# OpenGene/gencore

Hardware: AMD Instinct MI355X
Metric: consensus read-pairs/sec (whole node) + clustering HBM GB/s vs roofline (higher is better)
Workload: dtype u8

## Files before the change

### gencore_amd/csrc/engine.hip

```cpp
#include <hip/hip_runtime.h>
#include <hip/hip_ext.h>
#include <cstdio>
#include <cstdlib>
#include <algorithm>
#include <cstring>
#include <ctime>
#include <string>
#include <vector>

#include "gce_kernels.hpp"
#include "gce_pair2.hpp"
#include "gce_vote.hpp"
#include "gce_deep.hpp"
#include "gce_output.hpp"
#include "gce_depth.hpp"
#include "gce_inflate.hpp"
#include "gce_deflate.hpp"

namespace {

static thread_local double t_alloc_s = 0.0; static thread_local long t_alloc_n = 0; static thread_local size_t t_alloc_bytes = 0;
static inline double mono_s() { struct timespec ts; clock_gettime(CLOCK_MONOTONIC, &ts); return (double)ts.tv_sec + 1e-9 * (double)ts.tv_nsec; }
long long g_dev_live = 0, g_dev_peak = 0;
static int64_t g_pass_idx_ctr[4] = {0, 0, 0, 0};
// ... 466 lines not shown
    return GCE_OK;
}

__global__ __launch_bounds__(256) void k_publish_si(const StreamInfo *si, StreamInfo *host, unsigned long long *flag, unsigned long long seq) {
    const uint32_t *src = reinterpret_cast<const uint32_t *>(si);
    uint32_t *dst = reinterpret_cast<uint32_t *>(host);
    for (unsigned i = threadIdx.x; i < sizeof(StreamInfo) / 4; i += 256) dst[i] = src[i];
    __threadfence_system();
    __syncthreads();
    if (threadIdx.x == 0) __hip_atomic_store(flag, seq, __ATOMIC_RELEASE, __HIP_MEMORY_SCOPE_SYSTEM);
}
static_assert(sizeof(StreamInfo) % 4 == 0, "k_publish_si copies words");
static int read_si_begin(gce_engine *e, unsigned long long *seq_out) {
    *seq_out = 0;
    static const bool sync_copy = getenv("GCE_SYNC_COPY") != nullptr;
    if (!sync_copy && !e->si_pin) {
        void *hp = nullptr;
        if (hipHostMalloc(&hp, sizeof(StreamInfo) + 64, hipHostMallocMapped | hipHostMallocCoherent | hipHostMallocPortable) == hipSuccess) {
            void *dp = nullptr;
            if (hipHostGetDevicePointer(&dp, hp, 0) == hipSuccess) { memset(hp, 0, sizeof(StreamInfo) + 64); e->si_pin = hp; e->si_pin_dev = dp; }
            else (void)hipHostFree(hp);
        }
        (void)hipGetLastError();
    }
    if (!sync_copy && e->si_pin) {
        unsigned long long *dflag = reinterpret_cast<unsigned long long *>(reinterpret_cast<char *>(e->si_pin_dev) + ((sizeof(StreamInfo) + 7) & ~size_t(7)));
        const unsigned long long seq = ++e->si_seq;
        hipLaunchKernelGGL(k_publish_si, dim3(1), dim3(256), 0, e->stream, (const StreamInfo *)e->si.p, reinterpret_cast<StreamInfo *>(e->si_pin_dev), dflag, seq);
        HIPCHK(hipGetLastError());
        *seq_out = seq;
    }
    return GCE_OK;
}
static int read_si_end(gce_engine *e, unsigned long long seq) {
    bool published = false;
    if (seq) {
        StreamInfo *hs = reinterpret_cast<StreamInfo *>(e->si_pin);
        unsigned long long *hflag = reinterpret_cast<unsigned long long *>(reinterpret_cast<char *>(e->si_pin) + ((sizeof(StreamInfo) + 7) & ~size_t(7)));
        for (unsigned spins = 1;; spins++) {
            if (__atomic_load_n(hflag, __ATOMIC_ACQUIRE) == seq) { published = true; break; }
            if ((spins & 0x3FFF) == 0) {
                const hipError_t q = hipStreamQuery(e->stream);
                if (q == hipSuccess) { published = __atomic_load_n(hflag, __ATOMIC_ACQUIRE) == seq; break; }
                if (q != hipErrorNotReady) HIPCHK(q);
            }
            __builtin_ia32_pause();
        }
        if (published) memcpy(&e->h_si, hs, sizeof(StreamInfo));
    }
    if (!published) {
        HIPCHK(hipMemcpyAsync(&e->h_si, e->si.p, sizeof(StreamInfo), hipMemcpyDeviceToHost, e->stream));
        HIPCHK(hipStreamSynchronize(e->stream));
    }
    for (int k = 0; k < 6; k++) for (int q = 0; q < GCE_PRE_SLOTS; q++) { e->h_si.pre[k] += e->h_si.pre_slot[q][k]; e->h_si.post[k] += e->h_si.post_slot[q][k]; }
    if (e->h_si.err_key != ~0ull) { e->dev_error = -(int)(e->h_si.err_key & 0xFF); e->dev_error_read = (uint32_t)(e->h_si.err_key >> 8); }
    return GCE_OK;
}
static int read_si(gce_engine *e) {
    unsigned long long seq = 0;
    const int rc = read_si_begin(e, &seq);
    return rc != GCE_OK ? rc : read_si_end(e, seq);
}

static inline unsigned cdiv(uint64_t a, uint64_t b) { return (unsigned)((a + b - 1) / b); }
static const bool g_record_events = getenv("GCE_RECORD_EVENTS") != nullptr;
#define LAUNCH_EV(kernel, grid, block, stream, ev, ...) do { \
    if (g_record_events) { hipLaunchKernelGGL(kernel, grid, block, 0, stream, __VA_ARGS__); (void)hipEventRecord(ev, stream); } \
    else hipExtLaunchKernelGGL(kernel, grid, block, 0, stream, nullptr, ev, 0, __VA_ARGS__); } while (0)

struct FillSeg { void *p; uint64_t bytes; uint32_t val; uint32_t pad; };
struct FillArgs { FillSeg s[6]; };
__global__ __launch_bounds__(256) void k_fill_many(FillArgs a) {
    const FillSeg g = a.s[blockIdx.y];
    const uint64_t n16 = g.bytes >> 4;
    const uint32_t v = g.val * 0x01010101u;
    uint4 *q = reinterpret_cast<uint4 *>(g.p);
    for (uint64_t i = (uint64_t)blockIdx.x * 256 + threadIdx.x; i < n16; i += (uint64_t)gridDim.x * 256) q[i] = make_uint4(v, v, v, v);
    if (blockIdx.x == 0 && threadIdx.x < (g.bytes & 15)) reinterpret_cast<uint8_t *>(g.p)[(n16 << 4) + threadIdx.x] = (uint8_t)g.val;
}
static void fill_many(hipStream_t s, std::initializer_list<FillSeg> segs) {
    FillArgs a{}; int n = 0; uint64_t mx = 0;
    for (const FillSeg &g : segs) { a.s[n++] = g; mx = std::max<uint64_t>(mx, g.bytes); }
    const unsigned gx = (unsigned)std::min<uint64_t>(std::max<uint64_t>((mx >> 4) / (256 * 8), 1), 2048);
    hipLaunchKernelGGL(k_fill_many, dim3(gx, (unsigned)n), dim3(256), 0, s, a);
}

static int aux_ready(gce_engine *e) {
    if (e->aux_stream) return GCE_OK;
// ... 139 lines not shown
        int cb = 1; while (cb < 33 && (1ull << cb) <= (uint64_t)N + 1024) cb++;
        int qb = 1; while (qb < 52 && (1ull << qb) <= qmax) qb++;
        p.nw_cb = cb; p.nw_bd = 62 - cb - qb; p.nw_ok = !e->target_len.empty() && p.nw_bd >= 1;
        if (p.nw_bd > 40) p.nw_bd = 40;
    }
    const size_t qual_bytes = hb.qual_bytes ? hb.qual_bytes : 1;
    const size_t nsb1 = (size_t)(n_sblk > 0 ? n_sblk : 1);
#define ENS(buf, bytes) HIPCHK(e->buf.ensure(bytes))
    ENS(uinfo, n1 * 8); ENS(rdesc, n1 * sizeof(ReadDescP)); ENS(spatch, n1 * 4); ENS(slot, n1 * 4 + 16); ENS(score, qual_bytes + 64);
    ENS(out_flag, n1 + 144);        ENS(nmx, n1 * 4); ENS(orec, n1 * sizeof(OutRec)); ENS(out_index, n1 * 4);
    ENS(lrec, nsb1 * SB_READS * sizeof(LeadRec)); ENS(lout, nsb1 * SB_READS * sizeof(LeadOut));
    ENS(bhdr, nsb1 * sizeof(BlkHdr)); ENS(blk_base, nsb1 * 4);
    ENS(ev_tid, (size_t)max_events * 4); ENS(ev_pos, (size_t)max_events * 4); ENS(ev_read, (size_t)max_events * 4);
    ENS(table, T * sizeof(TabEntry)); ENS(toff, T * 4);
    ENS(k64, n1 * 24); ENS(members, n1 * 4); ENS(sorted, n1 * 4); ENS(pl, n1 * 4); ENS(pr, n1 * 4); ENS(pu, n1 * 4); ENS(pg, n1 * 4); ENS(gpl, n1 * 4); ENS(gpr, n1 * 4);
    ENS(grp_begin, n1 * 4); ENS(grp_n, n1 * 4); ENS(slow_list, n1 * 4 + 64);
    w.slow_list = e->slow_list.as<uint32_t>();
    ENS(deep_list, (n1 / 64 + 64) * 16); w.deep_list = e->deep_list.p;
    const unsigned nblk_N = cdiv(n1, SCAN_TILE);
    ENS(scan_part, std::max<size_t>(2 * nsb1, (size_t)2 * nblk_N) * 8 + 16);     ENS(si, sizeof(StreamInfo));
    w.uinfo = e->uinfo.as<uint64_t>(); w.rdesc = e->rdesc.as<ReadDescP>(); w.spatch = e->spatch.as<uint32_t>();
    w.slot = e->slot.as<uint32_t>(); w.score = e->score.as<int8_t>();
    w.out_flag = e->out_flag.as<uint8_t>(); w.nmx = e->nmx.as<uint32_t>(); w.orec = e->orec.as<OutRec>(); w.out_index = e->out_index.as<uint32_t>();
    w.lrec = e->lrec.as<LeadRec>(); w.lout = e->lout.as<LeadOut>(); w.bhdr = e->bhdr.as<BlkHdr>(); w.blk_base = e->blk_base.as<uint32_t>();
    w.ev_tid = e->ev_tid.as<int32_t>(); w.ev_pos = e->ev_pos.as<int32_t>(); w.ev_read = e->ev_read.as<uint32_t>();
    w.tab = e->table.as<TabEntry>(); w.toff = e->toff.as<uint32_t>();
    w.k64 = e->k64.as<uint64_t>(); w.members = e->members.as<uint32_t>(); w.sorted = e->sorted.as<uint32_t>(); w.pl = e->pl.as<uint32_t>(); w.pr = e->pr.as<uint32_t>();
    w.pu = e->pu.as<uint32_t>(); w.pg = e->pg.as<uint32_t>(); w.gpl = e->gpl.as<uint32_t>(); w.gpr = e->gpr.as<uint32_t>();
    w.grp_begin = e->grp_begin.as<uint32_t>(); w.grp_n = e->grp_n.as<uint32_t>();
    w.scan_part = e->scan_part.as<uint64_t>(); w.si = e->si.as<StreamInfo>();
    ENS(cl_ikey, n1 * 4); ENS(cl_start, n1 * 4); ENS(cl_n, n1 * 4);
    w.cl_ikey = e->cl_ikey.as<uint32_t>(); w.cl_start = e->cl_start.as<uint32_t>(); w.cl_n = e->cl_n.as<uint32_t>();

    StreamInfo init{}; init.first_unmapped = NONE32; init.err_key = ~0ull; init.lq_min = 0x7FFFFFFF; init.lq_max = -1;
    if (e->have_tick) { init.n_events = init.n_events_a = (int)e->h_ev_tid.size(); }
    HIPCHK(hipMemcpyAsync(e->si.p, &init, sizeof init, hipMemcpyHostToDevice, e->stream));
    if (e->have_tick && !e->h_ev_tid.empty()) {
        HIPCHK(hipMemcpyAsync(e->ev_tid.p, e->h_ev_tid.data(), e->h_ev_tid.size() * 4, hipMemcpyHostToDevice, e->stream));
        HIPCHK(hipMemcpyAsync(e->ev_pos.p, e->h_ev_pos.data(), e->h_ev_pos.size() * 4, hipMemcpyHostToDevice, e->stream));
    }
    hipStream_t s = e->stream;
    if (!e->tab_clean || e->tab_clean_ptr != e->table.p || e->tab_clean_cap != e->table.cap) {
        HIPCHK(hipMemsetAsync(e->table.p, 0, e->table.cap, s));
        e->tab_clean_ptr = e->table.p; e->tab_clean_cap = e->table.cap;
    }
    e->tab_clean = false;
    HIPCHK(hipEventRecord(e->ev[EV_START], s));
    HIPCHK(hipMemsetAsync(e->out_flag.p, 0, n1, s));
    if (N > 0) LAUNCH_EV(k_cluster, dim3((unsigned)n_sblk), dim3(SB_T), s, e->ev[EV_CLUSTER], b, p, w);
#ifdef CL_PROF
    if (N > 0) {
        StreamInfo hs; (void)hipStreamSynchronize(s); (void)hipMemcpy(&hs, e->si.p, sizeof hs, hipMemcpyDeviceToHost);
        static const char *nm[3] = {"key records + keys", "LDS leaders", "stores"};
        const double blocks = (double)hs.prof[15];
        fprintf(stderr, "k_cluster phases, mean per block (us), %.0f blocks:", blocks);
        for (int k = 0; k < 3; k++) fprintf(stderr, " %s %.2f;", nm[k], blocks ? hs.prof[k] / blocks / 100.0 : 0.0);
        fprintf(stderr, "\n");
    }
#endif
    if (N <= 0) HIPCHK(hipEventRecord(e->ev[EV_CLUSTER], s));
    CANARY("EV_CLUSTER");
    if (N > 0) {
        if (!e->have_tick) {
            hipLaunchKernelGGL(k_blk_scan, dim3(1), dim3(1024), 0, s, w, p);
            hipLaunchKernelGGL(k_events, dim3(cdiv(max_events, EV_T / 64)), dim3(EV_T), 0, s, b, p, w);
        }
        const unsigned nb4 = cdiv(n_sblk, 4);
        hipLaunchKernelGGL(k_leaders, dim3(nb4), dim3(256), 0, s, b, p, w);
        hipLaunchKernelGGL(k_num_reduce, dim3(nb4), dim3(256), 0, s, w, p.nw_cb);
        hipLaunchKernelGGL(k_scan_partials, dim3(1), dim3(1024), 0, s, w.scan_part, (uint64_t)nb4, &w.si->n_clusters, (unsigned long long *)nullptr);
        hipLaunchKernelGGL(k_num_apply, dim3(nb4), dim3(256), 0, s, w);
        LAUNCH_EV(k_scatter, dim3((unsigned)n_sblk), dim3(SB_T), s, e->ev[EV_CSR], N, w);
    } else HIPCHK(hipEventRecord(e->ev[EV_CSR], s));
    CANARY("EV_CSR");
    unsigned long long si_seq1 = 0;
    if ((rc = read_si_begin(e, &si_seq1)) != GCE_OK) return rc;
    if (N > 0) {
#ifndef GCE_DESCRIBE_BLOCKS
#define GCE_DESCRIBE_BLOCKS 32768
#endif
        const int64_t n_tiles = (N + 255) / 256;
        int tpb = (int)((n_tiles + GCE_DESCRIBE_BLOCKS - 1) / GCE_DESCRIBE_BLOCKS); if (tpb < 1) tpb = 1;
        LAUNCH_EV(k_describe, dim3(cdiv(n_tiles, tpb)), dim3(256), s, e->ev[EV_DESCRIBE], b, p, w, tpb);
    } else HIPCHK(hipEventRecord(e->ev[EV_DESCRIBE], s));
    CANARY("EV_DESCRIBE");
    if ((rc = read_si_end(e, si_seq1)) != GCE_OK) return rc;
    HIPCHK(hipGetLastError());
    e->tab_clean = true;
    const uint32_t C = (uint32_t)e->h_si.n_clusters;
    const size_t c1 = C ? C : 1;
    ENS(cl_npairs, c1 * 4); ENS(cl_ngroups, c1 * 4); ENS(cl_gbase, c1 * 4); ENS(cl_nresult, c1 * 4); ENS(cl_hasumi, c1); ENS(cl_tier, c1);
    w.cl_npairs = e->cl_npairs.as<uint32_t>(); w.cl_ngroups = e->cl_ngroups.as<uint32_t>(); w.cl_gbase = e->cl_gbase.as<uint32_t>();
    w.cl_nresult = e->cl_nresult.as<uint32_t>(); w.cl_hasumi = e->cl_hasumi.as<uint8_t>(); w.cl_tier = e->cl_tier.as<uint8_t>();
    uint32_t NG = 0;
    bool si_behind_describe = false;
    if (C > 0 && e->dev_error == 0) {
        ENS(left_list, c1 * 4 + 64); w.left_list = e->left_list.as<uint32_t>();
        ENS(pf_flag, c1 + 64); ENS(pf_list, c1 * 4); ENS(pq_flag, c1 + 64); ENS(pq_list, c1 * 4); ENS(p16_flag, c1 + 64); ENS(p16_list, c1 * 4);
        w.pf_flag = e->pf_flag.as<uint8_t>(); w.pf_list = e->pf_list.as<uint32_t>(); w.pq_flag = e->pq_flag.as<uint8_t>(); w.pq_list = e->pq_list.as<uint32_t>(); w.p16_flag = e->p16_flag.as<uint8_t>(); w.p16_list = e->p16_list.as<uint32_t>();
        const bool pair_classes = (double)N > 10.0 * (double)C;
        if (!pair_classes) fill_many(s, {FillSeg{e->pf_flag.p, c1, 0u, 0u}, FillSeg{e->pq_flag.p, c1, 0u, 0u}});
        const unsigned nbc = cdiv(C, SCAN_TILE);
        auto compact = [&](uint8_t *flag, uint32_t *list, unsigned long long *count) {
            hipLaunchKernelGGL(k_flag_reduce, dim3(nbc), dim3(256), 0, s, (const uint8_t *)flag, (uint64_t)C, w.scan_part);
            hipLaunchKernelGGL(k_scan_partials, dim3(1), dim3(1024), 0, s, w.scan_part, (uint64_t)nbc, count, (unsigned long long *)nullptr);
            hipLaunchKernelGGL(k_flag_apply, dim3(nbc), dim3(256), 0, s, (const uint8_t *)flag, (uint64_t)C, (const uint64_t *)w.scan_part, list);
        };
#ifdef PS_STOP
        {
            hipEvent_t a_, b_, c_; (void)hipEventCreate(&a_); (void)hipEventCreate(&b_); (void)hipEventCreate(&c_);
            (void)hipEventRecord(a_, s);
            hipLaunchKernelGGL(k_pairing_sub<16>, dim3(cdiv(C, 4 * WAVES_PER_BLOCK)), dim3(256), 0, s, b, p, w, C, (const uint32_t *)nullptr, (const unsigned long long *)nullptr, w.pq_flag, 0);
            (void)hipEventRecord(b_, s);
            hipLaunchKernelGGL(k_pairing_sub<32>, dim3(cdiv(C, 2 * WAVES_PER_BLOCK)), dim3(256), 0, s, b, p, w, C, (const uint32_t *)nullptr, (const unsigned long long *)nullptr, w.pf_flag, 0);
            (void)hipEventRecord(c_, s); (void)hipEventSynchronize(c_);
            float m1 = 0, m2 = 0; (void)hipEventElapsedTime(&m1, a_, b_); (void)hipEventElapsedTime(&m2, b_, c_);
            fprintf(stderr, "k_pairing_sub up to tick %d: <16> %.3f ms, <32> over ALL clusters %.3f ms\n", PS_STOP, m1, m2);
            return fail(e, GCE_ERR_INVALID, "experiment build");
        }
#endif
        ENS(pd_slab, PD_BIG_BLOCKS * PD_SLAB);
        if (pair_classes) {
            hipLaunchKernelGGL(k_pair_class_reduce, dim3(nbc), dim3(256), 0, s, (const uint32_t *)w.cl_n, C, w.scan_part);
            hipLaunchKernelGGL(k_scan_partials, dim3(1), dim3(1024), 0, s, w.scan_part, (uint64_t)nbc, &w.si->n_p16_items, &w.si->n_pq_items);
            hipLaunchKernelGGL(k_pair_class_apply, dim3(nbc), dim3(256), 0, s, (const uint32_t *)w.cl_n, C, (const uint64_t *)w.scan_part, w.p16_list, w.pq_list, w.pf_list, w.si);
            static const bool tiers_aux = getenv("GCE_NO_AUX_STREAM") == nullptr;
            hipStream_t s2 = s;
            if (tiers_aux) {
                if ((rc = aux_ready(e)) != GCE_OK) return rc;
                s2 = e->aux_stream;
                HIPCHK(hipEventRecord(e->aux_ev[0], s));
                HIPCHK(hipStreamWaitEvent(s2, e->aux_ev[0], 0));
            }
            hipLaunchKernelGGL(k_pairing_fast, dim3(2048), dim3(256), 0, s2, b, p, w, C, (const uint32_t *)w.pf_list);
            hipLaunchKernelGGL(k_pairing_deep<false>, dim3(256), dim3(PD_T), 0, s2, b, p, w, (uint8_t *)nullptr);
            if (tiers_aux) HIPCHK(hipEventRecord(e->aux_ev[1], s2));
            hipLaunchKernelGGL(k_pairing_sub<16>, dim3(cdiv(C, 4 * WAVES_PER_BLOCK)), dim3(256), 0, s, b, p, w, C, (const uint32_t *)w.p16_list, (const unsigned long long *)&w.si->n_p16_items, w.pq_flag, 1);
            hipLaunchKernelGGL(k_pairing_sub<32>, dim3(cdiv(C, 2 * WAVES_PER_BLOCK)), dim3(256), 0, s, b, p, w, C, (const uint32_t *)w.pq_list, (const unsigned long long *)&w.si->n_pq_items, w.pf_flag, 1);
            if (tiers_aux) HIPCHK(hipStreamWaitEvent(s, e->aux_ev[1], 0));
        } else {
            hipLaunchKernelGGL(k_pairing_sub<16>, dim3(cdiv(C, 4 * WAVES_PER_BLOCK)), dim3(256), 0, s, b, p, w, C, (const uint32_t *)nullptr, (const unsigned long long *)nullptr, w.pq_flag, 0);
            compact(w.pq_flag, w.pq_list, &w.si->n_pq_items);
            hipLaunchKernelGGL(k_pairing_sub<32>, dim3(cdiv(C, 2 * WAVES_PER_BLOCK)), dim3(256), 0, s, b, p, w, C, (const uint32_t *)w.pq_list, (const unsigned long long *)&w.si->n_pq_items, w.pf_flag, 0);
            compact(w.pf_flag, w.pf_list, &w.si->n_pf_items);
            hipLaunchKernelGGL(k_pairing_fast, dim3(2048), dim3(256), 0, s, b, p, w, C, (const uint32_t *)w.pf_list);
            hipLaunchKernelGGL(k_pairing_deep<false>, dim3(256), dim3(PD_T), 0, s, b, p, w, (uint8_t *)nullptr);
        }
        hipLaunchKernelGGL(k_pairing_deep<true>, dim3(PD_BIG_BLOCKS), dim3(PD_T), 0, s, b, p, w, e->pd_slab.as<uint8_t>());
        hipLaunchKernelGGL(k_pairing_slow<0>, dim3(1024), dim3(256), 0, s, b, p, w);
        hipLaunchKernelGGL(k_pairing_slow<1>, dim3(1024, 16), dim3(256), 0, s, b, p, w);
        hipLaunchKernelGGL(k_pairing_slow<2>, dim3(1024), dim3(256), 0, s, b, p, w);
        const unsigned nblk_C = cdiv(C, SCAN_TILE);
        hipLaunchKernelGGL(k_scan_reduce, dim3(nblk_C), dim3(256), 0, s, (const uint32_t *)w.cl_ngroups, (uint64_t)C, w.scan_part);
        hipLaunchKernelGGL(k_scan_partials, dim3(1), dim3(1024), 0, s, w.scan_part, (uint64_t)nblk_C, &w.si->n_pairs , &w.si->n_groups);
        hipLaunchKernelGGL(k_u32_apply, dim3(nblk_C), dim3(256), 0, s, (const uint32_t *)w.cl_ngroups, w.cl_gbase, (uint64_t)C, (const uint64_t *)w.scan_part);
        ENS(gl_cluster, n1 * 4); ENS(g_begin, n1 * 4); ENS(g_np, n1 * 4); ENS(gw, n1 * 8); ENS(g_wbase, n1 * 4);
        const size_t vb_cap = ((VB_MINW + 3) * n1) / VB_W + 8;
        ENS(vb_start, vb_cap * 4);
        w.gl_cluster = e->gl_cluster.as<uint32_t>(); w.g_begin = e->g_begin.as<uint32_t>(); w.g_np = e->g_np.as<uint32_t>();
        w.gw = e->gw.as<uint64_t>(); w.g_wbase = e->g_wbase.as<uint32_t>(); w.vb_start = e->vb_start.as<uint32_t>();
        HIPCHK(hipMemsetAsync(e->vb_start.p, 0xFF, vb_cap * 4, s));
        hipLaunchKernelGGL(k_group_fill, dim3(cdiv(C, 256)), dim3(256), 0, s, w, C, p.skip_low_complexity_thr, (uint32_t)VB_W, (uint32_t)VB_MINW);
        hipLaunchKernelGGL(k_u64_reduce, dim3(nblk_N), dim3(256), 0, s, (const uint64_t *)w.gw, (const unsigned long long *)&w.si->n_groups, w.scan_part);
        hipLaunchKernelGGL(k_u64_partials, dim3(1), dim3(1024), 0, s, w.scan_part, (const unsigned long long *)&w.si->n_groups, &w.si->vote_weight);
        LAUNCH_EV(k_vote_batches, dim3(nblk_N), dim3(256), s, e->ev[EV_PAIRING], w, (const unsigned long long *)&w.si->n_groups, (const uint64_t *)w.scan_part);
        CANARY("EV_PAIRING");
        if ((rc = read_si(e)) != GCE_OK) return rc;
        HIPCHK(hipGetLastError());
        si_behind_describe = true;
        NG = (uint32_t)e->h_si.n_groups;
    } else HIPCHK(hipEventRecord(e->ev[EV_PAIRING], s));
    const size_t g1 = NG ? NG : 1;
    ENS(gen_list, g1 * 8); ENS(gen_flag, g1 * 2 + 64); ENS(score_list, n1 * 4 + 64);       ENS(rp_left, g1 * 4); ENS(rp_right, g1 * 4); ENS(rp_merge, g1 * 4); ENS(rp_rmerge, g1 * 4); ENS(rp_umi, g1 * 8);
    ENS(rp_umilen, g1 * 2); ENS(rp_state, g1); ENS(rp_supp, g1 * 4); ENS(rp_nm, g1 * 8); ENS(rp_qsl, g1 * 4); ENS(rp_qsr, g1 * 4);
    w.gen_list = e->gen_list.as<uint32_t>(); w.gen_flag = e->gen_flag.as<uint8_t>(); w.score_list = e->score_list.as<uint32_t>();
    w.rp_left = e->rp_left.as<uint32_t>(); w.rp_right = e->rp_right.as<uint32_t>();
    w.rp_merge = e->rp_merge.as<uint32_t>(); w.rp_rmerge = e->rp_rmerge.as<uint32_t>(); w.rp_umi = e->rp_umi.as<const char *>();
    w.rp_umilen = e->rp_umilen.as<uint16_t>(); w.rp_state = e->rp_state.as<uint8_t>(); w.rp_supp = e->rp_supp.as<int32_t>();
    w.rp_nm = e->rp_nm.as<int32_t>(); w.rp_qsl = e->rp_qsl.as<uint32_t>(); w.rp_qsr = e->rp_qsr.as<uint32_t>();
    if (NG > 0 && e->dev_error == 0) {
        {
            SlowArgs sa; sa.b = b; sa.p = p; sa.w = w;
            HIPCHK(e->slow_args.ensure(sizeof sa));
            HIPCHK(hipMemcpyAsync(e->slow_args.p, &sa, sizeof sa, hipMemcpyHostToDevice, s));
        }
        fill_many(s, {FillSeg{e->gen_flag.p, g1 * 2, 0u, 0u},
                      FillSeg{e->rp_nm.p, g1 * 8, 0xFFu, 0u},
                      FillSeg{e->rp_left.p, g1 * 4, 0xFFu, 0u}, FillSeg{e->rp_right.p, g1 * 4, 0xFFu, 0u}});
#ifdef VB_XCD
        const unsigned nbatch = (((unsigned)(e->h_si.vote_weight / VB_W) + 1u) + 7u) & ~7u;
#else
        const unsigned nbatch = (unsigned)(e->h_si.vote_weight / VB_W) + 1u;
#endif
#ifdef VB_STOP
        {
            hipEvent_t a_, b_; (void)hipEventCreate(&a_); (void)hipEventCreate(&b_);
            (void)hipEventRecord(a_, s); hipLaunchKernelGGL(k_vote, dim3(nbatch), dim3(VB_T), 0, s, b, p, w, NG); (void)hipEventRecord(b_, s); (void)hipEventSynchronize(b_);
            float ms_ = 0; (void)hipEventElapsedTime(&ms_, a_, b_); fprintf(stderr, "k_vote up to tick %d: %.3f ms\n", VB_STOP, ms_);
            return fail(e, GCE_ERR_INVALID, "experiment build");
        }
#endif
        LAUNCH_EV(k_vote, dim3(nbatch), dim3(VB_T), s, e->ev[EV_SCORE], b, p, w, NG);
        CANARY("EV_SCORE");
        const bool deep_stream = ((double)N > 48.0 * (double)NG || getenv("GCE_FORCE_AUX_STREAM")) && !getenv("GCE_NO_AUX_STREAM");
// ... 37 lines not shown
#ifndef VB_COUNT
        fprintf(stderr, " [of P2: (a) reads vs class %.2f; (b) sides' states %.2f; the rest = order, prefixes, barrier]", blocks ? hs.prof[11] / blocks / 100.0 : 0.0, blocks ? hs.prof[12] / blocks / 100.0 : 0.0);
#endif
        fprintf(stderr, "\n");
#ifdef VB_COUNT
        fprintf(stderr, "k_vote columns in the full vote: %.0f, one base only: %.0f, of those unchanged: %.0f\n", (double)hs.prof[11], (double)hs.prof[12], (double)hs.prof[13]);
#endif
#ifdef DV_PROF
        fprintf(stderr, "k_deep_prepare: %.0f sides, mean %.1f us per side, mean %.0f pairs per side\n", (double)hs.prof[14], hs.prof[14] ? hs.prof[6] / (double)hs.prof[14] / 100.0 : 0.0, hs.prof[14] ? hs.prof[7] / (double)hs.prof[14] / 100.0 : 0.0);
#endif
        static const char *pn[8] = {"windows", "name sort", "pairs", "umi words", "umi sort", "grouping", "layout sort", "layout write"};
        const double cl = (double)hs.prof[30];
        fprintf(stderr, "k_pairing_deep phases, mean per cluster (us), %.0f clusters:", cl);
        for (int k = 0; k < 8; k++) fprintf(stderr, " %s %.1f;", pn[k], cl ? hs.prof[16 + k] / cl / 100.0 : 0.0);
        fprintf(stderr, "\n");
    }
#endif
    HIPCHK(hipEventRecord(e->ev[EV_FINISH], s));
    CANARY("EV_FINISH");
    OutTable o{};
    if (N > 0 && e->dev_error == 0) {
        size_t seq_cap = hb.seq_bytes + 16 * n1 + 64, qual_cap = hb.qual_bytes + 16 * n1 + 64;
        if (e->h_si.lq_max >= 0) {
            const size_t lqm = (size_t)e->h_si.lq_max;
            seq_cap = std::min(seq_cap, n1 * ((lqm + 1) / 2 + 16) + 64); qual_cap = std::min(qual_cap, n1 * (lqm + 16) + 64);
        }
        ENS(o_src, n1 * 4); ENS(o_kind, n1); ENS(o_qsrc, n1 * 4); ENS(o_nm, n1 * 4); ENS(o_fr, n1 * 2); ENS(o_rr, n1 * 2); ENS(o_mate, n1 * 4);
        ENS(o_soff, n1 * 8); ENS(o_qoff, n1 * 8); ENS(o_seq, seq_cap); ENS(o_qual, qual_cap);
        ENS(o_key, n1 * sizeof(OutKey)); ENS(o_rec, n1 * sizeof(OutRec)); ENS(o_ksoff, n1 * 8); ENS(o_kqoff, n1 * 8); ENS(o_krow, n1 * 4); ENS(o_rank64, (n1 / 64 + 2) * 4); const unsigned nblk_O = cdiv(n1, OUT_TILE); ENS(o_part3, (size_t)nblk_O * 24 + 64);
        o.src = e->o_src.as<uint32_t>(); o.kind = e->o_kind.as<uint8_t>(); o.qname_src = e->o_qsrc.as<uint32_t>(); o.nm_new = e->o_nm.as<int32_t>();
        o.fr = e->o_fr.as<int16_t>(); o.rr = e->o_rr.as<int16_t>(); o.mate = e->o_mate.as<uint32_t>();
        o.seq_off = e->o_soff.as<uint64_t>(); o.qual_off = e->o_qoff.as<uint64_t>(); o.seq = e->o_seq.as<uint8_t>(); o.qual = e->o_qual.as<uint8_t>();
        o.key = e->o_key.as<OutKey>(); o.rec = e->o_rec.as<OutRec>(); o.ksoff = e->o_ksoff.as<uint64_t>(); o.kqoff = e->o_kqoff.as<uint64_t>(); o.krow = e->o_krow.as<uint32_t>(); o.rank64 = e->o_rank64.as<uint32_t>(); o.part3 = e->o_part3.as<uint64_t>();
        hipLaunchKernelGGL(k_stats, dim3(1024), dim3(256), 0, s, b, w, (NG > 0 ? C : 0u), NG);
        CANARY("k_stats");
        hipLaunchKernelGGL(k_out_reduce, dim3(nblk_O), dim3(OUT_T), 0, s, b, w, o);
        CANARY("k_out_reduce");
        hipLaunchKernelGGL(k_out_partials, dim3(1), dim3(1024), 0, s, o, (uint64_t)nblk_O, w);
        CANARY("k_out_partials");
        const bool lq_uniform = si_behind_describe && e->h_si.lq_max >= 0 && e->h_si.lq_min == e->h_si.lq_max;
        if (lq_uniform) hipLaunchKernelGGL(k_out_meta<true>, dim3(nblk_O), dim3(OUT_T), 0, s, b, w, o, (int)e->h_si.lq_max);
        else hipLaunchKernelGGL(k_out_meta<false>, dim3(nblk_O), dim3(OUT_T), 0, s, b, w, o, -1);
        CANARY("k_out_meta");
        const unsigned og = std::min<unsigned>(cdiv(n1, 256), 8192u);
        hipLaunchKernelGGL(k_out_rows, dim3(og), dim3(256), 0, s, w, o);
        CANARY("k_out_rows");
        hipLaunchKernelGGL(k_out_mate, dim3(og), dim3(256), 0, s, w, o);
        CANARY("k_out_mate");
        hipLaunchKernelGGL(k_out_gather, dim3(std::min<unsigned>(cdiv(n1, 16), 16384u)), dim3(256), 0, s, b, w, o);
        CANARY("k_out_gather");
    }
    HIPCHK(hipEventRecord(e->ev[EV_OUTPUT], s));
    CANARY("EV_OUTPUT");
    hipLaunchKernelGGL(k_fold_stats, dim3(1), dim3(64), 0, s, w.si, pre_extra);
    if ((rc = read_si(e)) != GCE_OK) return rc;
    HIPCHK(hipGetLastError());
#ifdef GCE_SI_CHECK
    {
        bool badw = false;
        for (int k = 14; k < GCE_STATS_WORDS; k++) if ((k != 15 && e->h_si.post[k] != 0) || e->h_si.pre[k] < 0) badw = true;
        if (badw) {
            StreamInfo again; (void)hipMemcpy(&again, e->si.p, sizeof again, hipMemcpyDeviceToHost);
            fprintf(stderr, "SI_CHECK: N %lld NG %u C %u n_out %llu\n post:", (long long)N, NG, C, (unsigned long long)e->h_si.n_out);
            for (int k = 0; k < 30; k++) fprintf(stderr, " %lld", e->h_si.post[k]);
            fprintf(stderr, "\n post again:"); for (int k = 0; k < 30; k++) fprintf(stderr, " %lld", again.post[k]);
            fprintf(stderr, "\n pre:"); for (int k = 0; k < 30; k++) fprintf(stderr, " %lld", e->h_si.pre[k]);
            fprintf(stderr, "\n other nonzero post words:"); for (int k = 30; k < GCE_STATS_WORDS; k++) if (e->h_si.post[k]) fprintf(stderr, " [%d]=%lld", k, e->h_si.post[k]);
            fprintf(stderr, "\n post_slot col 0..7 sums:"); for (int k = 0; k < 8; k++) { long long a = 0; for (int q = 0; q < GCE_PRE_SLOTS; q++) a += e->h_si.post_slot[q][k]; fprintf(stderr, " %lld", a); }
            fprintf(stderr, "\n scalars: n_clustered %llu n_slow %u n_deep %u n_slow_pair %u n_gen %llu n_pf %llu n_pq %llu vote_weight %llu\n", e->h_si.n_clustered, e->h_si.n_slow, e->h_si.n_deep, e->h_si.n_slow_pair, (unsigned long long)(e->h_si.hand_on >> 32), e->h_si.n_pf_items, e->h_si.n_pq_items, e->h_si.vote_weight);
        }
    }
#endif
    e->h_si.n_groups = NG;
    float ms = 0;
    auto el = [&](int a, int c) { ms = 0; (void)hipEventElapsedTime(&ms, e->ev[a], e->ev[c]); return (double)ms; };
    e->timing.total_ms = el(EV_START, EV_OUTPUT);
    e->timing.cluster_ms = el(EV_START, EV_CLUSTER); e->timing.csr_ms = el(EV_CLUSTER, EV_CSR); e->timing.describe_ms = el(EV_CSR, EV_DESCRIBE);
    e->timing.pairing_ms = el(EV_DESCRIBE, EV_PAIRING); e->timing.score_ms = el(EV_PAIRING, EV_SCORE); e->timing.consensus_ms = el(EV_SCORE, EV_CONSENSUS);
    e->timing.finish_ms = el(EV_CONSENSUS, EV_FINISH); e->timing.output_ms = el(EV_FINISH, EV_OUTPUT);
    e->timing.n_clusters = C; e->timing.n_groups = NG;
    if (e->dev_error != 0) {
        char buf[160]; snprintf(buf, sizeof buf, "%s (read %u)", gce_status_message(e->dev_error), e->dev_error_read);
        return fail(e, e->dev_error, buf);
    }
    e->n_out = (int64_t)e->h_si.n_out;
    e->out_seq_bytes = (size_t)(e->h_si.out_units >> 32) * 16; e->out_qual_bytes = (size_t)(e->h_si.out_units & 0xFFFFFFFFull) * 16;
    e->timing.n_pairs = (int64_t)e->h_si.n_pairs_total; e->timing.n_leaders = (int64_t)e->h_si.n_leaders;
    return GCE_OK;
// ... 188 lines not shown
```

### gencore_amd/csrc/gce_cluster.hpp

```cpp
#pragma once

#ifndef SB_T
#define SB_T 512
#endif
#ifndef SB_U
#define SB_U 2
#endif
#define SB_READS (SB_T * SB_U)
#define SB_LDS_SLOTS (2 * SB_READS)
#define SB_OFF_BITS (SB_READS == 1024 ? 10 : 9)
static_assert(SB_READS == 512 || SB_READS == 1024, "LeadRec.info packs a place and a count of SB_READS");

struct __attribute__((aligned(16))) LeadRec { unsigned long long kw; uint32_t info, runlen; };
static_assert(sizeof(LeadRec) == 16, "LeadRec must stay 16 bytes");
#define LI_ODD (1u << 22)
struct __attribute__((aligned(8))) BlkHdr { uint32_t n_lead, n_clu; };
struct __attribute__((aligned(8))) LeadOut { uint32_t h, rb; };
#define LO_OWNER 0x80000000u

__device__ __forceinline__ uint32_t d_thr_mode(uint32_t ikey, const StreamInfo *si, const DevParams &p) {
    uint32_t inst = ikey & 0x7FFFFFFFu, seg_b = ikey >> 31;
    if (!seg_b) {
        if ((int)(inst + 1) <= si->n_events_a) return THR_PROPER;
        if (si->first_unmapped != NONE32) return THR_UNPROPER;
// ... 430 lines not shown
        uint64_t x = v;
        for (int o = 1; o < 64; o <<= 1) { uint64_t t = (uint64_t)__shfl_up((long long)x, o); if (lane >= o) x += t; }
        if (v) {
            const uint64_t ex = carry + x - v;
            const uint32_t cid = (uint32_t)(ex >> 32);
            w.cl_start[cid] = (uint32_t)ex; w.cl_n[cid] = (uint32_t)v; w.cl_ikey[cid] = (uint32_t)(ic >> 32); w.toff[h] = (uint32_t)ex;
        }
        carry += rl64(x, 63);
    }
}
__global__ __launch_bounds__(SB_T) void k_scatter(int64_t n, Work w) {
    __shared__ uint32_t s_dst[SB_READS];
    const int64_t blk = blockIdx.x;
    const uint32_t nl = w.bhdr[blk].n_lead;
    uint32_t v[SB_U];
#pragma unroll
    for (int u = 0; u < SB_U; u++) { const int64_t i = (blk * SB_U + u) * SB_T + threadIdx.x; v[u] = i < n ? w.slot[i] : NONE32; }
    for (uint32_t kq = threadIdx.x; kq < nl; kq += SB_T) {
        const LeadOut o = w.lout[(size_t)blk * SB_READS + kq];
        s_dst[kq] = w.toff[o.h] + (o.rb & ~LO_OWNER);
        if (o.rb & LO_OWNER) *reinterpret_cast<uint4 *>(&w.tab[o.h]) = make_uint4(0, 0, 0, 0);
    }
    __syncthreads();
#pragma unroll
    for (int u = 0; u < SB_U; u++) {
        const int64_t i = (blk * SB_U + u) * SB_T + threadIdx.x;
        if (v[u] != NONE32) w.members[s_dst[v[u] & 0xFFFFu] + (v[u] >> 16)] = (uint32_t)i;
    }
}

#ifndef DESC_WPE
#define DESC_WPE 8
#endif
__global__ __launch_bounds__(256, DESC_WPE) void k_describe(DevBatch b, DevParams p, Work w, int tiles_per_block) {
    __shared__ long long s_stat[WAVES_PER_BLOCK][6];
    long long st[6] = {0, 0, 0, 0, 0, 0};
    int lqmin = 0x7FFFFFFF, lqmax = -1;
    const int lane = lane_id(), wv = threadIdx.x >> 6;
    for (int cb = 0; cb < tiles_per_block; cb++) {
        const int64_t i = ((int64_t)blockIdx.x * tiles_per_block + cb) * 256 + threadIdx.x;
        if (i < b.n) {
            union { gce_core c; uint4 q[2]; } t; const uint4 *src = reinterpret_cast<const uint4 *>(b.core + i); t.q[0] = src[0]; t.q[1] = src[1];
            const gce_core k = t.c;
            const uint8_t c = d_classify(k);
            bool mapped = k.tid >= 0;
            const int nmv = b.nm[i]; const bool has_nm = b.nm_type[i] != 0;
            int mism = (mapped && has_nm) ? nmv : 0;
            w.nmx[i] = ((uint32_t)nmv << 1) | (has_nm ? 1u : 0u);
            st[0] += 1; st[1] += k.l_qseq; st[4] += mism;
            if (!mapped) { st[2] += 1; st[3] += k.l_qseq; }
            if (mism > 0) st[5] += 1;
            if (c != CLS_DROP) { lqmin = min(lqmin, k.l_qseq); lqmax = max(lqmax, k.l_qseq); }
            if (c == CLS_CLUSTERED) {
                const uint32_t *cg = b.cigar + b.cigar_off[i];
                const uint32_t c0w = k.n_cigar ? cg[0] : 0;
                int mo_ = 0, ml_ = 0;
                if (k.n_cigar == 1) ml_ = cig_op(c0w) == 0 ? cig_len(c0w) : 0;
                else d_first_m(cg, k.n_cigar, mo_, ml_);
                if (k.l_qseq > 65535) raise_error(w.si, GCE_ERR_INVALID, (uint32_t)i);
                if (p.ref_win && k.isize != 0 && k.tid < p.n_ref && p.ref_data[k.tid]) {
                    const int64_t rl = k.n_cigar == 1 ? (int64_t)cig_len(c0w) * consumes_ref(cig_op(c0w)) : (int64_t)d_cigar_rlen(cg, k.n_cigar);
                    const int64_t end_in = min((int64_t)k.pos + rl, p.ref_len[k.tid]);
                    if ((int64_t)k.pos < p.ref_win[2 * k.tid] || end_in > p.ref_win[2 * k.tid + 1]) raise_error(w.si, GCE_ERR_REF_WINDOW, (uint32_t)i);
                }
                store_desc(w.rdesc, (uint64_t)i, b.seq_off[i], b.qual_off[i], c0w, k.pos, k.isize != 0, k.l_qseq, mo_, ml_, k.n_cigar, k.tid, k.n_cigar > 1 ? cg[k.n_cigar - 1] : c0w);
                const char *src2; uint8_t hm = 0;
                if (b.mi && b.mi_off[i] != 0xFFFFFFFFFFFFFFFFull) { src2 = b.mi + b.mi_off[i]; hm = 1; }
                else src2 = b.qname + b.qname_off[i];
                int s0, l0;
                if (!d_umi_slice(src2, p, s0, l0, hm ? -1 : (int)k.l_qname - 1)) { raise_error(w.si, GCE_ERR_UMI_PARSE, (uint32_t)i); s0 = 0; l0 = 0; }
                if (l0 > UINFO_MAXLEN) { raise_error(w.si, GCE_ERR_UMI_PARSE, (uint32_t)i); l0 = 0; }
                w.uinfo[i] = uinfo_pack((hm ? b.mi_off[i] : b.qname_off[i]) + (uint64_t)s0, hm != 0, k.l_qname, l0);
            }
        }
    }
    for (int k = 0; k < 6; k++) { long long v = wave_sum64(st[k]); if (lane == 0) s_stat[wv][k] = v; }
    lqmin = wave_min(lqmin); lqmax = wave_max(lqmax);
    if (lane == 0) {
        if (lqmin < *(volatile int *)&w.si->lq_min) atomicMin(&w.si->lq_min, lqmin);
        if (lqmax > *(volatile int *)&w.si->lq_max) atomicMax(&w.si->lq_max, lqmax);
    }
    __syncthreads();
    if (threadIdx.x < 6) {
        long long v = s_stat[0][threadIdx.x] + s_stat[1][threadIdx.x] + s_stat[2][threadIdx.x] + s_stat[3][threadIdx.x];
        if (v) atomicAdd((unsigned long long *)&w.si->pre_slot[blockIdx.x & (GCE_PRE_SLOTS - 1)][threadIdx.x], (unsigned long long)v);
    }
}
```

### gencore_amd/csrc/gce_device.hpp

```cpp
#pragma once
#include <hip/hip_runtime.h>
#include <stdint.h>
#include "../../include/gencore_amd.h"

#define GCE_WAVE 64
#define NONE32 0xFFFFFFFFu
#define EMPTY64 0xFFFFFFFFFFFFFFFFull

enum : uint32_t { THR_PROPER = 0, THR_UNPROPER = 1, THR_NEVER = 2 };
enum : uint8_t { TIER_NEVER = 0, TIER_SUB16 = 1, TIER_SUB32 = 2, TIER_FAST = 3, TIER_DEEP_LDS = 4, TIER_DEEP_DEVICE = 5, TIER_GENERIC = 6 };
enum : uint8_t { CLS_DROP = 0, CLS_CLUSTERED = 1, CLS_BYPASS = 2 };

struct DevBatch {
    int64_t n;
    const gce_core *core;
    const uint64_t *qname_off; const char *qname;
    const uint64_t *cigar_off; const uint32_t *cigar;
    const uint64_t *seq_off;   uint8_t *seq;
    const uint64_t *qual_off;  uint8_t *qual;
    const int32_t *nm; const uint8_t *nm_type;
    const uint64_t *mi_off; const char *mi;
    const uint64_t *tick;
};

// ... 24 lines not shown
    const int64_t *ref_win;
};

#define GCE_PRE_SLOTS 64
struct StreamInfo {
    unsigned long long n_clustered;
    unsigned int first_unmapped;
    unsigned long long err_key;
    int n_events;
    int n_events_a;
    unsigned int n_slow;
    unsigned long long prof[32];
    unsigned int n_deep;
    unsigned long long hand_on;
    unsigned int n_slow_pair;
    unsigned int n_slow_pair2;
    unsigned int pair_next, pair_next2;
    unsigned int prep_next, deep_next;
    int lq_min, lq_max;
    unsigned long long n_clusters, n_groups, n_pairs, n_out;
    unsigned long long n_pairs_total;
    unsigned long long vote_weight;
    unsigned long long n_leaders;
    unsigned long long out_units;
    unsigned long long n_pf_items;
    unsigned long long n_pq_items;
    unsigned long long n_p16_items;
    unsigned long long vote_rounds2;
    unsigned long long vote_rounds2_unaligned;
    long long pre[GCE_STATS_WORDS];
    long long post[GCE_STATS_WORDS];
    long long post_slot[GCE_PRE_SLOTS][8];
    long long pre_slot[GCE_PRE_SLOTS][8];
};

__device__ __forceinline__ void raise_error(StreamInfo *si, int code, uint32_t read) {
    atomicMin(&si->err_key, ((unsigned long long)read << 8) | (unsigned long long)((-code) & 0xFF));
}

__device__ __forceinline__ int lane_id() { return threadIdx.x & 63; }

__device__ __forceinline__ int cig_op(uint32_t w) { return (int)(w & 0xF); }
__device__ __forceinline__ int cig_len(uint32_t w) { return (int)(w >> 4); }
__device__ __forceinline__ int consumes_query(int op) { return (0x193 >> op) & 1; }
__device__ __forceinline__ int consumes_ref(int op) { return (0x18D >> op) & 1; }

struct __attribute__((aligned(16))) ReadDescP {
    uint32_t so_lo, qo_lo;
    uint32_t c0;
    uint32_t pos_fl;
    uint16_t lq, mo, ml, nc;
    int32_t tid;
    uint32_t hi;
};
static_assert(sizeof(ReadDescP) == 32, "ReadDescP must stay 32 bytes");
struct ReadDesc {
    uint64_t so, qo;
    uint32_t c0;
    int32_t pos, lq, isize;
    int32_t mo, ml;
    int32_t tid;
    uint16_t nc, lastm;
    int32_t rlen;
};
#define RLEN_WALK (-0x40000000)
__device__ __forceinline__ void store_desc(ReadDescP *base, uint64_t i, uint64_t so, uint64_t qo, uint32_t c0, int32_t pos, bool isize_nz, int lq, int mo, int ml, int nc, int32_t tid, uint32_t last_op) {
    union { ReadDescP d; uint4 q[2]; } u;
    u.d.so_lo = (uint32_t)so; u.d.qo_lo = (uint32_t)qo; const uint32_t lastm = cig_op(last_op) == 0 ? min((uint32_t)cig_len(last_op), 65535u) : 0u;
    u.d.hi = ((uint32_t)(so >> 32) & 0xFFu) | ((uint32_t)(qo >> 32) & 0xFFu) << 8 | lastm << 16;
    u.d.c0 = c0; u.d.pos_fl = (uint32_t)pos | (isize_nz ? 0x80000000u : 0u);
// ... 343 lines not shown
```

Baseline: 1.826 billion.

## Split describe kernel and overlap its parts and output kernels on an aux stream

Splits k_describe into a UMI-slicing kernel and a descriptor/stats kernel. The UMI part now runs on an auxiliary stream concurrently with clustering, and the descriptor part runs alongside pairing, joining before the vote batches. k_out_rows, k_out_mate and k_stats are also moved to the aux stream so they overlap k_out_gather. The early stream-info read is moved before k_num_apply so the host can pick up the cluster count sooner. To keep errors raised by the concurrently running describe kernels from being seen too early, they go to a separate err_key_desc field. The cost is extra cross-stream events, a second pass over core records, and concurrency that now depends on correct event ordering.

```diff
diff --git a/gencore_amd/csrc/engine.hip b/gencore_amd/csrc/engine.hip
--- a/gencore_amd/csrc/engine.hip
+++ b/gencore_amd/csrc/engine.hip
@@ -522,7 +522,7 @@
     }
     return GCE_OK;
 }
-static int read_si_end(gce_engine *e, unsigned long long seq) {
+static int read_si_end(gce_engine *e, unsigned long long seq, bool first_look = false) {
     bool published = false;
     if (seq) {
         StreamInfo *hs = reinterpret_cast<StreamInfo *>(e->si_pin);
@@ -543,7 +543,9 @@
         HIPCHK(hipStreamSynchronize(e->stream));
     }
     for (int k = 0; k < 6; k++) for (int q = 0; q < GCE_PRE_SLOTS; q++) { e->h_si.pre[k] += e->h_si.pre_slot[q][k]; e->h_si.post[k] += e->h_si.post_slot[q][k]; }
-    if (e->h_si.err_key != ~0ull) { e->dev_error = -(int)(e->h_si.err_key & 0xFF); e->dev_error_read = (uint32_t)(e->h_si.err_key >> 8); }
+    if (first_look) { e->h_si.err_key_desc = ~0ull; e->h_si.lq_min = 0x7FFFFFFF; e->h_si.lq_max = -1; }
+    const unsigned long long ek = std::min(e->h_si.err_key, e->h_si.err_key_desc);
+    if (ek != ~0ull) { e->dev_error = -(int)(ek & 0xFF); e->dev_error_read = (uint32_t)(ek >> 8); }
     return GCE_OK;
 }
 static int read_si(gce_engine *e) {
@@ -749,7 +751,7 @@
     ENS(cl_ikey, n1 * 4); ENS(cl_start, n1 * 4); ENS(cl_n, n1 * 4);
     w.cl_ikey = e->cl_ikey.as<uint32_t>(); w.cl_start = e->cl_start.as<uint32_t>(); w.cl_n = e->cl_n.as<uint32_t>();
 
-    StreamInfo init{}; init.first_unmapped = NONE32; init.err_key = ~0ull; init.lq_min = 0x7FFFFFFF; init.lq_max = -1;
+    StreamInfo init{}; init.first_unmapped = NONE32; init.err_key = ~0ull; init.err_key_desc = ~0ull; init.lq_min = 0x7FFFFFFF; init.lq_max = -1;
     if (e->have_tick) { init.n_events = init.n_events_a = (int)e->h_ev_tid.size(); }
     HIPCHK(hipMemcpyAsync(e->si.p, &init, sizeof init, hipMemcpyHostToDevice, e->stream));
     if (e->have_tick && !e->h_ev_tid.empty()) {
@@ -763,6 +765,46 @@
     }
     e->tab_clean = false;
     HIPCHK(hipEventRecord(e->ev[EV_START], s));
+#ifndef GCE_OVL_UMI
+#define GCE_OVL_UMI 1
+#endif
+#ifndef GCE_OVL_DESC
+#define GCE_OVL_DESC 1
+#endif
+#ifndef GCE_OVL_ROWS
+#define GCE_OVL_ROWS 1
+#endif
+#ifndef GCE_OVL_STATS
+#define GCE_OVL_STATS 1
+#endif
+    static const bool use_aux = getenv("GCE_NO_AUX_STREAM") == nullptr;
+    struct AuxGuard { gce_engine *e; bool armed; ~AuxGuard() { if (armed && e->aux_stream) (void)hipStreamSynchronize(e->aux_stream); } } aux_guard{e, false};
+#ifndef GCE_DESCRIBE_BLOCKS
+#define GCE_DESCRIBE_BLOCKS 32768
+#endif
+    const int64_t n_tiles = (N + 255) / 256;
+    int tpb = (int)((n_tiles + GCE_DESCRIBE_BLOCKS - 1) / GCE_DESCRIBE_BLOCKS); if (tpb < 1) tpb = 1;
+    bool umi_forked = false, desc_forked = false;
+    auto fork_desc = [&]() -> int {
+        if (N <= 0 || desc_forked || !(use_aux && GCE_OVL_DESC)) return GCE_OK;
+        const int rc2 = aux_ready(e); if (rc2 != GCE_OK) return rc2;
+        HIPCHK(hipStreamWaitEvent(e->aux_stream, e->ev[EV_CSR], 0));
+        hipLaunchKernelGGL(k_describe_desc, dim3(cdiv(n_tiles, tpb)), dim3(256), 0, e->aux_stream, b, p, w, tpb);
+        HIPCHK(hipEventRecord(e->aux_ev[3], e->aux_stream));
+        desc_forked = true; aux_guard.armed = true;
+        return GCE_OK;
+    };
+    auto join_desc = [&]() -> int {
+        if (desc_forked) { HIPCHK(hipStreamWaitEvent(s, e->aux_ev[3], 0)); desc_forked = false; }
+        return GCE_OK;
+    };
+    if (N > 0 && use_aux && GCE_OVL_UMI) {
+        if ((rc = aux_ready(e)) != GCE_OK) return rc;
+        HIPCHK(hipStreamWaitEvent(e->aux_stream, e->ev[EV_START], 0));
+        hipLaunchKernelGGL(k_describe_umi, dim3((unsigned)n_tiles), dim3(256), 0, e->aux_stream, b, p, w);
+        HIPCHK(hipEventRecord(e->aux_ev[2], e->aux_stream));
+        umi_forked = true; aux_guard.armed = true;
+    }
     HIPCHK(hipMemsetAsync(e->out_flag.p, 0, n1, s));
     if (N > 0) LAUNCH_EV(k_cluster, dim3((unsigned)n_sblk), dim3(SB_T), s, e->ev[EV_CLUSTER], b, p, w);
 #ifdef CL_PROF
@@ -777,6 +819,7 @@
 #endif
     if (N <= 0) HIPCHK(hipEventRecord(e->ev[EV_CLUSTER], s));
     CANARY("EV_CLUSTER");
+    unsigned long long si_seq1 = 0;
     if (N > 0) {
         if (!e->have_tick) {
             hipLaunchKernelGGL(k_blk_scan, dim3(1), dim3(1024), 0, s, w, p);
@@ -786,22 +829,20 @@
         hipLaunchKernelGGL(k_leaders, dim3(nb4), dim3(256), 0, s, b, p, w);
         hipLaunchKernelGGL(k_num_reduce, dim3(nb4), dim3(256), 0, s, w, p.nw_cb);
         hipLaunchKernelGGL(k_scan_partials, dim3(1), dim3(1024), 0, s, w.scan_part, (uint64_t)nb4, &w.si->n_clusters, (unsigned long long *)nullptr);
+        if ((rc = read_si_begin(e, &si_seq1)) != GCE_OK) return rc;
         hipLaunchKernelGGL(k_num_apply, dim3(nb4), dim3(256), 0, s, w);
         LAUNCH_EV(k_scatter, dim3((unsigned)n_sblk), dim3(SB_T), s, e->ev[EV_CSR], N, w);
     } else HIPCHK(hipEventRecord(e->ev[EV_CSR], s));
     CANARY("EV_CSR");
-    unsigned long long si_seq1 = 0;
-    if ((rc = read_si_begin(e, &si_seq1)) != GCE_OK) return rc;
+    if (N <= 0 && (rc = read_si_begin(e, &si_seq1)) != GCE_OK) return rc;
     if (N > 0) {
-#ifndef GCE_DESCRIBE_BLOCKS
-#define GCE_DESCRIBE_BLOCKS 32768
-#endif
-        const int64_t n_tiles = (N + 255) / 256;
-        int tpb = (int)((n_tiles + GCE_DESCRIBE_BLOCKS - 1) / GCE_DESCRIBE_BLOCKS); if (tpb < 1) tpb = 1;
-        LAUNCH_EV(k_describe, dim3(cdiv(n_tiles, tpb)), dim3(256), s, e->ev[EV_DESCRIBE], b, p, w, tpb);
+        if (umi_forked) HIPCHK(hipStreamWaitEvent(s, e->aux_ev[2], 0));
+        else hipLaunchKernelGGL(k_describe_umi, dim3((unsigned)n_tiles), dim3(256), 0, s, b, p, w);
+        if (use_aux && GCE_OVL_DESC) HIPCHK(hipEventRecord(e->ev[EV_DESCRIBE], s));
+        else LAUNCH_EV(k_describe_desc, dim3(cdiv(n_tiles, tpb)), dim3(256), s, e->ev[EV_DESCRIBE], b, p, w, tpb);
     } else HIPCHK(hipEventRecord(e->ev[EV_DESCRIBE], s));
     CANARY("EV_DESCRIBE");
-    if ((rc = read_si_end(e, si_seq1)) != GCE_OK) return rc;
+    if ((rc = read_si_end(e, si_seq1, true)) != GCE_OK) return rc;
     HIPCHK(hipGetLastError());
     e->tab_clean = true;
     const uint32_t C = (uint32_t)e->h_si.n_clusters;
@@ -816,6 +857,10 @@
         ENS(pf_flag, c1 + 64); ENS(pf_list, c1 * 4); ENS(pq_flag, c1 + 64); ENS(pq_list, c1 * 4); ENS(p16_flag, c1 + 64); ENS(p16_list, c1 * 4);
         w.pf_flag = e->pf_flag.as<uint8_t>(); w.pf_list = e->pf_list.as<uint32_t>(); w.pq_flag = e->pq_flag.as<uint8_t>(); w.pq_list = e->pq_list.as<uint32_t>(); w.p16_flag = e->p16_flag.as<uint8_t>(); w.p16_list = e->p16_list.as<uint32_t>();
         const bool pair_classes = (double)N > 10.0 * (double)C;
+#ifndef GCE_DESC_FRONT
+#define GCE_DESC_FRONT 1
+#endif
+        if (GCE_DESC_FRONT && (rc = fork_desc()) != GCE_OK) return rc;
         if (!pair_classes) fill_many(s, {FillSeg{e->pf_flag.p, c1, 0u, 0u}, FillSeg{e->pq_flag.p, c1, 0u, 0u}});
         const unsigned nbc = cdiv(C, SCAN_TILE);
         auto compact = [&](uint8_t *flag, uint32_t *list, unsigned long long *count) {
@@ -852,10 +897,12 @@
             hipLaunchKernelGGL(k_pairing_fast, dim3(2048), dim3(256), 0, s2, b, p, w, C, (const uint32_t *)w.pf_list);
             hipLaunchKernelGGL(k_pairing_deep<false>, dim3(256), dim3(PD_T), 0, s2, b, p, w, (uint8_t *)nullptr);
             if (tiers_aux) HIPCHK(hipEventRecord(e->aux_ev[1], s2));
+            if ((rc = fork_desc()) != GCE_OK) return rc;
             hipLaunchKernelGGL(k_pairing_sub<16>, dim3(cdiv(C, 4 * WAVES_PER_BLOCK)), dim3(256), 0, s, b, p, w, C, (const uint32_t *)w.p16_list, (const unsigned long long *)&w.si->n_p16_items, w.pq_flag, 1);
             hipLaunchKernelGGL(k_pairing_sub<32>, dim3(cdiv(C, 2 * WAVES_PER_BLOCK)), dim3(256), 0, s, b, p, w, C, (const uint32_t *)w.pq_list, (const unsigned long long *)&w.si->n_pq_items, w.pf_flag, 1);
             if (tiers_aux) HIPCHK(hipStreamWaitEvent(s, e->aux_ev[1], 0));
         } else {
+            if ((rc = fork_desc()) != GCE_OK) return rc;
             hipLaunchKernelGGL(k_pairing_sub<16>, dim3(cdiv(C, 4 * WAVES_PER_BLOCK)), dim3(256), 0, s, b, p, w, C, (const uint32_t *)nullptr, (const unsigned long long *)nullptr, w.pq_flag, 0);
             compact(w.pq_flag, w.pq_list, &w.si->n_pq_items);
             hipLaunchKernelGGL(k_pairing_sub<32>, dim3(cdiv(C, 2 * WAVES_PER_BLOCK)), dim3(256), 0, s, b, p, w, C, (const uint32_t *)w.pq_list, (const unsigned long long *)&w.si->n_pq_items, w.pf_flag, 0);
@@ -880,13 +927,18 @@
         hipLaunchKernelGGL(k_group_fill, dim3(cdiv(C, 256)), dim3(256), 0, s, w, C, p.skip_low_complexity_thr, (uint32_t)VB_W, (uint32_t)VB_MINW);
         hipLaunchKernelGGL(k_u64_reduce, dim3(nblk_N), dim3(256), 0, s, (const uint64_t *)w.gw, (const unsigned long long *)&w.si->n_groups, w.scan_part);
         hipLaunchKernelGGL(k_u64_partials, dim3(1), dim3(1024), 0, s, w.scan_part, (const unsigned long long *)&w.si->n_groups, &w.si->vote_weight);
+        if ((rc = join_desc()) != GCE_OK) return rc;
         LAUNCH_EV(k_vote_batches, dim3(nblk_N), dim3(256), s, e->ev[EV_PAIRING], w, (const unsigned long long *)&w.si->n_groups, (const uint64_t *)w.scan_part);
         CANARY("EV_PAIRING");
         if ((rc = read_si(e)) != GCE_OK) return rc;
         HIPCHK(hipGetLastError());
         si_behind_describe = true;
         NG = (uint32_t)e->h_si.n_groups;
-    } else HIPCHK(hipEventRecord(e->ev[EV_PAIRING], s));
+    } else {
+        if ((rc = fork_desc()) != GCE_OK) return rc;
+        if ((rc = join_desc()) != GCE_OK) return rc;
+        HIPCHK(hipEventRecord(e->ev[EV_PAIRING], s));
+    }
     const size_t g1 = NG ? NG : 1;
     ENS(gen_list, g1 * 8); ENS(gen_flag, g1 * 2 + 64); ENS(score_list, n1 * 4 + 64);       ENS(rp_left, g1 * 4); ENS(rp_right, g1 * 4); ENS(rp_merge, g1 * 4); ENS(rp_rmerge, g1 * 4); ENS(rp_umi, g1 * 8);
     ENS(rp_umilen, g1 * 2); ENS(rp_state, g1); ENS(rp_supp, g1 * 4); ENS(rp_nm, g1 * 8); ENS(rp_qsl, g1 * 4); ENS(rp_qsr, g1 * 4);
@@ -990,7 +1042,8 @@
         o.fr = e->o_fr.as<int16_t>(); o.rr = e->o_rr.as<int16_t>(); o.mate = e->o_mate.as<uint32_t>();
         o.seq_off = e->o_soff.as<uint64_t>(); o.qual_off = e->o_qoff.as<uint64_t>(); o.seq = e->o_seq.as<uint8_t>(); o.qual = e->o_qual.as<uint8_t>();
         o.key = e->o_key.as<OutKey>(); o.rec = e->o_rec.as<OutRec>(); o.ksoff = e->o_ksoff.as<uint64_t>(); o.kqoff = e->o_kqoff.as<uint64_t>(); o.krow = e->o_krow.as<uint32_t>(); o.rank64 = e->o_rank64.as<uint32_t>(); o.part3 = e->o_part3.as<uint64_t>();
-        hipLaunchKernelGGL(k_stats, dim3(1024), dim3(256), 0, s, b, w, (NG > 0 ? C : 0u), NG);
+        const bool ovl_rows = use_aux && GCE_OVL_ROWS, ovl_stats = use_aux && GCE_OVL_STATS;
+        if (!ovl_stats) hipLaunchKernelGGL(k_stats, dim3(1024), dim3(256), 0, s, b, w, (NG > 0 ? C : 0u), NG);
         CANARY("k_stats");
         hipLaunchKernelGGL(k_out_reduce, dim3(nblk_O), dim3(OUT_T), 0, s, b, w, o);
         CANARY("k_out_reduce");
@@ -1001,17 +1054,29 @@
         else hipLaunchKernelGGL(k_out_meta<false>, dim3(nblk_O), dim3(OUT_T), 0, s, b, w, o, -1);
         CANARY("k_out_meta");
         const unsigned og = std::min<unsigned>(cdiv(n1, 256), 8192u);
-        hipLaunchKernelGGL(k_out_rows, dim3(og), dim3(256), 0, s, w, o);
+        hipStream_t s3 = s;
+        if (ovl_rows || ovl_stats) {
+            if ((rc = aux_ready(e)) != GCE_OK) return rc;
+            s3 = e->aux_stream;
+            HIPCHK(hipEventRecord(e->aux_ev[0], s));
+            HIPCHK(hipStreamWaitEvent(s3, e->aux_ev[0], 0));
+            aux_guard.armed = true;
+        }
+        hipLaunchKernelGGL(k_out_rows, dim3(og), dim3(256), 0, ovl_rows ? s3 : s, w, o);
         CANARY("k_out_rows");
-        hipLaunchKernelGGL(k_out_mate, dim3(og), dim3(256), 0, s, w, o);
+        hipLaunchKernelGGL(k_out_mate, dim3(og), dim3(256), 0, ovl_rows ? s3 : s, w, o);
         CANARY("k_out_mate");
+        if (ovl_stats) hipLaunchKernelGGL(k_stats, dim3(1024), dim3(256), 0, s3, b, w, (NG > 0 ? C : 0u), NG);
+        if (s3 != s) HIPCHK(hipEventRecord(e->aux_ev[1], s3));
         hipLaunchKernelGGL(k_out_gather, dim3(std::min<unsigned>(cdiv(n1, 16), 16384u)), dim3(256), 0, s, b, w, o);
         CANARY("k_out_gather");
+        if (s3 != s) HIPCHK(hipStreamWaitEvent(s, e->aux_ev[1], 0));
     }
     HIPCHK(hipEventRecord(e->ev[EV_OUTPUT], s));
     CANARY("EV_OUTPUT");
     hipLaunchKernelGGL(k_fold_stats, dim3(1), dim3(64), 0, s, w.si, pre_extra);
     if ((rc = read_si(e)) != GCE_OK) return rc;
+    aux_guard.armed = false;
     HIPCHK(hipGetLastError());
 #ifdef GCE_SI_CHECK
     {
diff --git a/gencore_amd/csrc/gce_cluster.hpp b/gencore_amd/csrc/gce_cluster.hpp
--- a/gencore_amd/csrc/gce_cluster.hpp
+++ b/gencore_amd/csrc/gce_cluster.hpp
@@ -486,7 +486,21 @@
 #ifndef DESC_WPE
 #define DESC_WPE 8
 #endif
-__global__ __launch_bounds__(256, DESC_WPE) void k_describe(DevBatch b, DevParams p, Work w, int tiles_per_block) {
+__global__ __launch_bounds__(256) void k_describe_umi(DevBatch b, DevParams p, Work w) {
+    const int64_t i = (int64_t)blockIdx.x * 256 + threadIdx.x;
+    if (i >= b.n) return;
+    union { gce_core c; uint4 q[2]; } t; const uint4 *src = reinterpret_cast<const uint4 *>(b.core + i); t.q[0] = src[0]; t.q[1] = src[1];
+    if (d_classify(t.c) != CLS_CLUSTERED) return;
+    const int l_qname = t.c.l_qname;
+    const char *src2; uint8_t hm = 0;
+    if (b.mi && b.mi_off[i] != 0xFFFFFFFFFFFFFFFFull) { src2 = b.mi + b.mi_off[i]; hm = 1; }
+    else src2 = b.qname + b.qname_off[i];
+    int s0, l0;
+    if (!d_umi_slice(src2, p, s0, l0, hm ? -1 : l_qname - 1)) { raise_error_desc(w.si, GCE_ERR_UMI_PARSE, (uint32_t)i); s0 = 0; l0 = 0; }
+    if (l0 > UINFO_MAXLEN) { raise_error_desc(w.si, GCE_ERR_UMI_PARSE, (uint32_t)i); l0 = 0; }
+    w.uinfo[i] = uinfo_pack((hm ? b.mi_off[i] : b.qname_off[i]) + (uint64_t)s0, hm != 0, l_qname, l0);
+}
+__global__ __launch_bounds__(256, DESC_WPE) void k_describe_desc(DevBatch b, DevParams p, Work w, int tiles_per_block) {
     __shared__ long long s_stat[WAVES_PER_BLOCK][6];
     long long st[6] = {0, 0, 0, 0, 0, 0};
     int lqmin = 0x7FFFFFFF, lqmax = -1;
@@ -511,20 +525,13 @@
                 int mo_ = 0, ml_ = 0;
                 if (k.n_cigar == 1) ml_ = cig_op(c0w) == 0 ? cig_len(c0w) : 0;
                 else d_first_m(cg, k.n_cigar, mo_, ml_);
-                if (k.l_qseq > 65535) raise_error(w.si, GCE_ERR_INVALID, (uint32_t)i);
+                if (k.l_qseq > 65535) raise_error_desc(w.si, GCE_ERR_INVALID, (uint32_t)i);
                 if (p.ref_win && k.isize != 0 && k.tid < p.n_ref && p.ref_data[k.tid]) {
                     const int64_t rl = k.n_cigar == 1 ? (int64_t)cig_len(c0w) * consumes_ref(cig_op(c0w)) : (int64_t)d_cigar_rlen(cg, k.n_cigar);
                     const int64_t end_in = min((int64_t)k.pos + rl, p.ref_len[k.tid]);
-                    if ((int64_t)k.pos < p.ref_win[2 * k.tid] || end_in > p.ref_win[2 * k.tid + 1]) raise_error(w.si, GCE_ERR_REF_WINDOW, (uint32_t)i);
+                    if ((int64_t)k.pos < p.ref_win[2 * k.tid] || end_in > p.ref_win[2 * k.tid + 1]) raise_error_desc(w.si, GCE_ERR_REF_WINDOW, (uint32_t)i);
                 }
                 store_desc(w.rdesc, (uint64_t)i, b.seq_off[i], b.qual_off[i], c0w, k.pos, k.isize != 0, k.l_qseq, mo_, ml_, k.n_cigar, k.tid, k.n_cigar > 1 ? cg[k.n_cigar - 1] : c0w);
-                const char *src2; uint8_t hm = 0;
-                if (b.mi && b.mi_off[i] != 0xFFFFFFFFFFFFFFFFull) { src2 = b.mi + b.mi_off[i]; hm = 1; }
-                else src2 = b.qname + b.qname_off[i];
-                int s0, l0;
-                if (!d_umi_slice(src2, p, s0, l0, hm ? -1 : (int)k.l_qname - 1)) { raise_error(w.si, GCE_ERR_UMI_PARSE, (uint32_t)i); s0 = 0; l0 = 0; }
-                if (l0 > UINFO_MAXLEN) { raise_error(w.si, GCE_ERR_UMI_PARSE, (uint32_t)i); l0 = 0; }
-                w.uinfo[i] = uinfo_pack((hm ? b.mi_off[i] : b.qname_off[i]) + (uint64_t)s0, hm != 0, k.l_qname, l0);
             }
         }
     }
diff --git a/gencore_amd/csrc/gce_device.hpp b/gencore_amd/csrc/gce_device.hpp
--- a/gencore_amd/csrc/gce_device.hpp
+++ b/gencore_amd/csrc/gce_device.hpp
@@ -80,10 +80,14 @@
     long long post[GCE_STATS_WORDS];
     long long post_slot[GCE_PRE_SLOTS][8];
     long long pre_slot[GCE_PRE_SLOTS][8];
+    unsigned long long err_key_desc;
 };
 
 __device__ __forceinline__ void raise_error(StreamInfo *si, int code, uint32_t read) {
     atomicMin(&si->err_key, ((unsigned long long)read << 8) | (unsigned long long)((-code) & 0xFF));
+}
+__device__ __forceinline__ void raise_error_desc(StreamInfo *si, int code, uint32_t read) {
+    atomicMin(&si->err_key_desc, ((unsigned long long)read << 8) | (unsigned long long)((-code) & 0xFF));
 }
 
 __device__ __forceinline__ int lane_id() { return threadIdx.x & 63; }
```

New measurement: 1.778 billion, median of 2. -2.6%, worse.
